# fxxJuses/MICFormer

Measured on AMD Instinct MI355X. Metric: train volumes/sec (128^3 CT+MRI pair), higher is better.
Workload: dtype bf16; 1 GPU; MicFormer base Head(embed_dim=48, depths 2-2-6-2, heads 3-6-12-24, window 2^3, 8 classes) full train step (fwd + MDiceLoss + bwd + Adam/cosine) on 128^3 CT+MR pairs, DropPath on; local_batch=2, global_batch=2, parallelism=dp1, launch=hipGraph replay (one graph)

## Files before the change

### micformer_amd/csrc/common.h

```cpp
#pragma once
#include <hip/hip_runtime.h>
#include <stdint.h>

#include "../../include/micformer_hip.h"
#include "gemm_core.h"

#define MICF_RETURN_LAUNCH()                          \
  do {                                                \
    return hipGetLastError() == hipSuccess ? MICF_OK : MICF_ELAUNCH; \
  } while (0)

namespace micf {

struct Options {
  int block_wave = 1;
  int block_recompute_h = 0;
  int block_debug = 0;
  int sample_tile = 1;
  int sample_e = -1;
  int cell_cap = -1;
  int tile_cap_hits = -1, tile_cap_cell = -1, tile_cap_voxel = -1;
};
Options& options();

struct Geo {
  int B, D, H, W;
  FastDiv fW, fH, fD;
  Geo() {}
  Geo(int B_, int D_, int H_, int W_) : B(B_), D(D_), H(H_), W(W_), fW((uint32_t)W_), fH((uint32_t)H_), fD((uint32_t)D_) {}
  __host__ __device__ int64_t tokens() const { return (int64_t)B * D * H * W; }
  __device__ __forceinline__ void decode(int t, int& b, int& d, int& h, int& w) const {
    uint32_t q, r;
    fW.divmod((uint32_t)t, q, r); w = (int)r;
    fH.divmod(q, q, r); h = (int)r;
    fD.divmod(q, q, r); d = (int)r; b = (int)q;
  }
  __device__ __forceinline__ int token(int b, int d, int h, int w) const { return ((b * D + d) * H + h) * W + w; }
};

__device__ __forceinline__ float wave_sum(float v) {
#pragma unroll
  for (int o = 32; o > 0; o >>= 1) v += __shfl_xor(v, o, 64);
  return v;
}

int colsum_atomic(const float* dy, const float* scale, int64_t rps, float* out, int64_t M, int N, hipStream_t s);

constexpr int kOffsetHidden = 16;
struct CellLists {
  int* count;
  int* ovf_count;
  int* list;
  int* ovf;
  int cap;
  float* w8;
};
struct SampleFwdSet { const float *h, *ln_g, *ln_b, *w1, *xa; float *flow, *xs; };
struct SampleBwdSet {
  const float *dxs, *h, *ln_g, *ln_b, *w1, *xa, *flow;
  float *dxa, *dh, *dln_g, *dln_b, *dw1;
  CellLists cl;
  float* partials;
};
int offset_sample_fwd_groups(const SampleFwdSet* sets, int n, int B, int D, int H, int W, int C, float eps, hipStream_t stream);
int offset_sample_bwd_groups(SampleBwdSet* sets, int n, int B, int D, int H, int W, int C, float eps, float* workspace,
                             int64_t workspace_floats, hipStream_t s, int phase = 0);
struct SampleFinishCall { const SampleBwdSet* sets; int n, B, D, H, W, C; float* workspace; int64_t workspace_floats; };
int offset_sample_finish_many(const SampleFinishCall* calls, int ncalls, hipStream_t s);

struct Conv3FwdSet { const float* x1; const float* x2; const float* w; const float* bias; float* y; float* wt; };
struct Conv3BwdSet { const float* dy; const float* w; float* wt; float* dx1; float* dx2; };
int conv3_fwd_x_groups(const Conv3FwdSet* sets, int n, int c1, int c2, int B, int D, int H, int W, int N, hipStream_t stream, int dtype,
                       int prepared, int y_zeroed);
bool conv3_fwd_x_splits(int B, int D, int H, int W, int c1, int c2);
int conv3_bwd_data_x_groups(const Conv3BwdSet* sets, int ng, int c1, int acc1, int c2, int acc2, int B, int D, int H, int W, int N,
                            hipStream_t stream, int dtype, int prepared);

int conv3_bwd_data_x(const float* dy, const float* w, float* wt, float* dx1, int c1, int acc1, float* dx2, int c2, int acc2, int B,
                     int D, int H, int W, int N, hipStream_t stream, int dtype = 0, int prepared = 0);

int64_t conv3_fwdx_workspace(int N, int c1, int c2);
int conv3_fwd_x(const float* x1, int c1, const float* x2, int c2, const float* w, const float* bias, float* y, float* wt, int B, int D,
                int H, int W, int N, hipStream_t stream, int dtype = 0, int prepared = 0);
int64_t conv3_wgradx_workspace(int B, int D, int H, int W, int N, int c1, int c2, int items = 1);
int conv3_wgradx_items(const float* const* dy, const float* const* x1, const float* const* x2, float* const* dw, float* const* dbias,
                       int n, int c1, int c2, int B, int D, int H, int W, int N, float* ws, int64_t ws_floats, hipStream_t stream,
                       int dtype);
int conv3_wgradx(const float* dy, const float* x1, int c1, const float* x2, int c2, float* dw, float* dbias, int B, int D, int H,
                 int W, int N, float* ws, int64_t ws_floats, hipStream_t stream, int dtype = 0);

}
```

### micformer_amd/csrc/conv3_wgradx.hip

```cpp
#include <cstdlib>
#include <mutex>

#include "common.h"
#include "gemm_dma.h"

namespace micf {

constexpr int wCS = 48;
constexpr int wDS = 20;
constexpr int wXS = 52;
constexpr int wPairs = 27 * (wCS / 16);
constexpr int wTPW = (wPairs + 3) / 4;
constexpr int wSlabFloats = 4 * wTPW * 256;

constexpr int kWgxItems = 12;
struct WgxArgs {
  const float* dy[kWgxItems];
  const float* x1[kWgxItems]; const float* x2[kWgxItems];
  int c1, c2;
  float* ws;
  float* bias_ws;
  int B, D, H, W, tiles_d, tiles_h, tiles_w, tiles_per_group, groups, slabs, xcd_order;
};

// ... 149 lines not shown

constexpr int wRSB = 104;
constexpr int wDYB = 40;
typedef short s16x4x __attribute__((ext_vector_type(4)));

__device__ __forceinline__ bf16x8 tr_pair(unsigned a0, unsigned a1) {
  const s16x4x lo = __builtin_amdgcn_ds_read_tr16_b64_v4i16((__attribute__((address_space(3))) s16x4x*)(uintptr_t)a0);
  const s16x4x hi = __builtin_amdgcn_ds_read_tr16_b64_v4i16((__attribute__((address_space(3))) s16x4x*)(uintptr_t)a1);
  return bf16x8{lo[0], lo[1], lo[2], lo[3], hi[0], hi[1], hi[2], hi[3]};
}

template <int TW>
__global__ void __launch_bounds__(256) conv3_wgradx_b16_kernel(WgxArgs a) {
  constexpr int TH = 64 / TW;
  constexpr int HH = TH + 2, HW = TW + 2, HALO = 3 * HH * HW;
  extern __shared__ __attribute__((aligned(16))) char smem[];
  const int tid = threadIdx.x, lane = tid & 63, wave = __builtin_amdgcn_readfirstlane(tid >> 6), li = lane & 15, lr = lane >> 4;
  int slab = blockIdx.x, group = blockIdx.y;
  const int item = blockIdx.z;
  if (a.xcd_order) {
    const int L = gridDim.x * gridDim.y;
    const int lin = slab + gridDim.x * group;
    const int logical = (lin % 8) * (L / 8) + lin / 8;
    slab = logical % gridDim.x;
    group = logical / gridDim.x;
  }
  const float* __restrict__ a_dy = a.dy[item];
  const float* __restrict__ a_x1 = a.x1[item];
  const float* __restrict__ a_x2 = a.x2[item];
  const int Cin = a.c1 + a.c2;
  const int cbase = slab * wCS;
  const int64_t DHW = (int64_t)a.D * a.H * a.W;
  const unsigned xh = (unsigned)(uintptr_t)smem, dyl = xh + HALO * wRSB;

  f32x4 acc[wTPW];
#pragma unroll
  for (int p = 0; p < wTPW; ++p) acc[p] = f32x4{0.f, 0.f, 0.f, 0.f};
  int offs[wTPW];
#pragma unroll
  for (int p = 0; p < wTPW; ++p) {
    const int pair = min(wave * wTPW + p, wPairs - 1);
    const int tap = pair / (wCS / 16), ct = pair % (wCS / 16);
    const int kd = tap / 9, kh = (tap / 3) % 3, kw = tap % 3;
    offs[p] = (((kd - 1) * HH + (kh - 1)) * HW + (kw - 1)) * wRSB + ct * 32;
  }
  unsigned abase[2][2], bbase[2][2];
#pragma unroll
  for (int ks = 0; ks < 2; ++ks)
#pragma unroll
    for (int r = 0; r < 2; ++r) {
      const int t = 8 * lr + 4 * r + (li >> 2);
      const int lh = ks * (32 / TW) + t / TW, lw = t % TW;
      abase[ks][r] = xh + (unsigned)(((1 * HH + lh + 1) * HW + lw + 1) * wRSB + 8 * (li & 3));
      bbase[ks][r] = dyl + (unsigned)((32 * ks + t) * wDYB + 8 * (li & 3));
    }
  float4 bs = make_float4(0.f, 0.f, 0.f, 0.f);

  const int ntiles = a.B * a.tiles_d * a.tiles_h * a.tiles_w;
  const int t_begin = group * a.tiles_per_group;
  const int t_end = min(ntiles, t_begin + a.tiles_per_group);
  constexpr int NQ = HALO * (wCS / 4);
  constexpr int NB = 16;
  static_assert(NQ <= 256 * NB, "one batch per tile");
  float4 v[NB], vdy;
  auto fetch = [&](int tile) {
    int q = tile;
    const int tw = q % a.tiles_w; q /= a.tiles_w;
    const int th = q % a.tiles_h; q /= a.tiles_h;
    const int d0 = q % a.tiles_d; const int b = q / a.tiles_d;
    const int h0 = th * TH, w0 = tw * TW;
#pragma unroll
    for (int u = 0; u < NB; ++u) {
      const int idx = u * 256 + tid;
      v[u] = make_float4(0.f, 0.f, 0.f, 0.f);
      if (idx < NQ) {
        const int hv = idx / (wCS / 4), g = idx % (wCS / 4);
        const int hw = hv % HW, hh = (hv / HW) % HH, hd = hv / (HW * HH);
        const int dd = d0 + hd - 1, yy = h0 + hh - 1, ww = w0 + hw - 1;
        const int c = cbase + 4 * g;
        if ((unsigned)dd < (unsigned)a.D && (unsigned)yy < (unsigned)a.H && (unsigned)ww < (unsigned)a.W && c < Cin) {
          const int64_t tok = (int64_t)b * DHW + ((int64_t)dd * a.H + yy) * a.W + ww;
          v[u] = c < a.c1 ? *reinterpret_cast<const float4*>(a_x1 + tok * a.c1 + c)
                          : *reinterpret_cast<const float4*>(a_x2 + tok * a.c2 + (c - a.c1));
        }
      }
    }
    const int tk = tid >> 2, yy = h0 + tk / TW, ww = w0 + tk % TW;
    vdy = make_float4(0.f, 0.f, 0.f, 0.f);
    if (yy < a.H && ww < a.W)
      vdy = *reinterpret_cast<const float4*>(a_dy + ((int64_t)b * DHW + ((int64_t)d0 * a.H + yy) * a.W + ww) * 16 + 4 * (tid & 3));
  };
  typedef unsigned u32x2w __attribute__((ext_vector_type(2)));
  if (t_begin < t_end) fetch(t_begin);
  for (int tile = t_begin; tile < t_end; ++tile) {
    __syncthreads();
#pragma unroll
    for (int u = 0; u < NB; ++u) {
      const int idx = u * 256 + tid;
      if (idx < NQ)
        *reinterpret_cast<u32x2w*>(smem + (idx / (wCS / 4)) * wRSB + 8 * (idx % (wCS / 4))) = u32x2w{pack_bf16(v[u].x, v[u].y), pack_bf16(v[u].z, v[u].w)};
    }
    *reinterpret_cast<u32x2w*>(smem + HALO * wRSB + (tid >> 2) * wDYB + 8 * (tid & 3)) = u32x2w{pack_bf16(vdy.x, vdy.y), pack_bf16(vdy.z, vdy.w)};
    bs.x += vdy.x; bs.y += vdy.y; bs.z += vdy.z; bs.w += vdy.w;
    __syncthreads();
    if (tile + 1 < t_end) fetch(tile + 1);
#pragma unroll
    for (int ks = 0; ks < 2; ++ks) {
      const bf16x8 bb = tr_pair(bbase[ks][0], bbase[ks][1]);
#pragma unroll
      for (int p = 0; p < wTPW; ++p) {
        const bf16x8 ba = tr_pair(abase[ks][0] + offs[p], abase[ks][1] + offs[p]);
        acc[p] = __builtin_amdgcn_mfma_f32_16x16x32_bf16(ba, bb, acc[p], 0, 0, 0);
      }
    }
  }
  float* out = a.ws + (((int64_t)item * a.slabs + slab) * a.groups + group) * wSlabFloats;
#pragma unroll
  for (int p = 0; p < wTPW; ++p)
    *reinterpret_cast<float4*>(out + ((wave * wTPW + p) * 64 + lane) * 4) = make_float4(acc[p][0], acc[p][1], acc[p][2], acc[p][3]);
  if (a.bias_ws && slab == 0) {
#pragma unroll
    for (int d = 4; d < 64; d <<= 1) {
      bs.x += __shfl_xor(bs.x, d, 64); bs.y += __shfl_xor(bs.y, d, 64); bs.z += __shfl_xor(bs.z, d, 64); bs.w += __shfl_xor(bs.w, d, 64);
    }
    __syncthreads();
    float* red = reinterpret_cast<float*>(smem);
    if (lane < 4) *reinterpret_cast<float4*>(red + (wave * 4 + lane) * 4) = bs;
    __syncthreads();
    if (tid < 16) a.bias_ws[((int64_t)item * a.groups + group) * 16 + tid] = red[tid] + red[16 + tid] + red[32 + tid] + red[48 + tid];
  }
}

struct WgxOut { float* dw[kWgxItems]; float* dbias[kWgxItems]; };
__global__ void __launch_bounds__(256) conv3_wgradx_reduce_kernel(const float* __restrict__ ws_all, const float* __restrict__ bias_all,
                                                                  WgxOut o, int Cin, int slabs, int groups) {
  __shared__ float red[256];
  const int item = blockIdx.y;
  const float* __restrict__ ws = ws_all + (int64_t)item * slabs * groups * wSlabFloats;
  const float* __restrict__ bias_ws = bias_all ? bias_all + (int64_t)item * groups * 16 : nullptr;
  float* __restrict__ dw = o.dw[item];
  float* __restrict__ dbias = o.dbias[item];
  const int el = threadIdx.x & 63, slice = threadIdx.x >> 6;
  const int64_t id = (int64_t)blockIdx.x * 64 + el;
  const int64_t per_slab = (int64_t)wPairs * 256;
  const bool main = id < per_slab * slabs;
  const bool bias = !main && bias_ws && dbias && id < per_slab * slabs + 16;
  float acc = 0.f;
  int slab = 0, e = 0;
  if (main) {
    slab = (int)(id / per_slab);
    e = (int)(id % per_slab);
    const float* p = ws + (int64_t)slab * groups * wSlabFloats + e;
    int g = slice;
    for (; g + 28 < groups; g += 32) {
      float v[8];
#pragma unroll
      for (int u = 0; u < 8; ++u) v[u] = p[(int64_t)(g + 4 * u) * wSlabFloats];
#pragma unroll
      for (int u = 0; u < 8; ++u) acc += v[u];
    }
    for (; g < groups; g += 4) acc += p[(int64_t)g * wSlabFloats];
  } else if (bias) {
    const int n = (int)(id - per_slab * slabs);
    for (int g = slice; g < groups; g += 4) acc += bias_ws[g * 16 + n];
  }
  red[threadIdx.x] = acc;
  __syncthreads();
  if (slice != 0) return;
  acc = red[el] + red[64 + el] + red[128 + el] + red[192 + el];
  if (main) {
    const int pair = e >> 8, lane = (e >> 2) & 63, v = e & 3;
    const int tap = pair / (wCS / 16), ct = pair % (wCS / 16);
    const int n = lane & 15, c = slab * wCS + ct * 16 + 4 * (lane >> 4) + v;
    if (c < Cin) dw[((int64_t)n * Cin + c) * 27 + tap] += acc;
  } else if (bias) {
    dbias[(int)(id - per_slab * slabs)] += acc;
  }
}

struct WgxPlan { int slabs, groups, tiles_per_group, tw; int64_t floats; };

static WgxPlan wgx_plan(int B, int D, int H, int W, int Cin, int items = 1) {
  WgxPlan p;
  p.tw = W >= 12 ? 16 : 8;
  const int th = 64 / p.tw;
  const int ntiles = B * D * ((H + th - 1) / th) * ((W + p.tw - 1) / p.tw);
  p.slabs = (Cin + wCS - 1) / wCS;
  constexpr int wg_target = 256;
  int groups = (wg_target + p.slabs * items - 1) / (p.slabs * items);
  if (groups < 4) groups = 4 < ntiles ? 4 : ntiles;
  if (groups > ntiles) groups = ntiles;
  p.tiles_per_group = (ntiles + groups - 1) / groups;
  p.groups = (ntiles + p.tiles_per_group - 1) / p.tiles_per_group;
  p.floats = (int64_t)p.slabs * p.groups * wSlabFloats + (int64_t)p.groups * 16;
  return p;
}

int64_t conv3_wgradx_workspace(int B, int D, int H, int W, int N, int c1, int c2, int items) {
  if (N != 16 || W < 4 || (c1 & 3) || (c2 & 3) || items < 1 || items > kWgxItems) return 0;
  return wgx_plan(B, D, H, W, c1 + c2, items).floats * items;
}

int conv3_wgradx_items(const float* const* dy, const float* const* x1, const float* const* x2, float* const* dw, float* const* dbias,
                       int n, int c1, int c2, int B, int D, int H, int W, int N, float* ws, int64_t ws_floats, hipStream_t stream,
                       int dtype) {
  const int64_t need = conv3_wgradx_workspace(B, D, H, W, N, c1, c2, n);
  if (need == 0 || !ws || ws_floats < need || !aligned16(ws)) return MICF_EUNSUPPORTED;
  const WgxPlan p = wgx_plan(B, D, H, W, c1 + c2, n);
  WgxArgs a{};
  WgxOut o{};
  bool any_bias = false;
  for (int i = 0; i < n; ++i) {
    if (!dy[i] || !x1[i] || !dw[i] || !aligned16(dy[i]) || !aligned16(x1[i]) || (x2 && x2[i] && !aligned16(x2[i]))) return MICF_EUNSUPPORTED;
    a.dy[i] = dy[i]; a.x1[i] = x1[i]; a.x2[i] = (x2 && x2[i]) ? x2[i] : x1[i];
    o.dw[i] = dw[i]; o.dbias[i] = dbias ? dbias[i] : nullptr;
    any_bias = any_bias || o.dbias[i];
  }
  a.c1 = c1; a.c2 = c2;
  a.ws = ws; a.bias_ws = any_bias ? ws + (int64_t)n * p.slabs * p.groups * wSlabFloats : nullptr;
  a.B = B; a.D = D; a.H = H; a.W = W;
  const int th = 64 / p.tw;
  a.tiles_d = D; a.tiles_h = (H + th - 1) / th; a.tiles_w = (W + p.tw - 1) / p.tw;
  a.tiles_per_group = p.tiles_per_group; a.groups = p.groups; a.slabs = p.slabs;
  a.xcd_order = ((p.slabs * p.groups) % 8 == 0) ? 1 : 0;
  static std::once_flag attr_once;
  std::call_once(attr_once, [] {
    (void)hipFuncSetAttribute(reinterpret_cast<const void*>(&conv3_wgradx_kernel<16, false>), hipFuncAttributeMaxDynamicSharedMemorySize, 80 * 1024);
    (void)hipFuncSetAttribute(reinterpret_cast<const void*>(&conv3_wgradx_kernel<8, false>), hipFuncAttributeMaxDynamicSharedMemorySize, 80 * 1024);
    (void)hipFuncSetAttribute(reinterpret_cast<const void*>(&conv3_wgradx_b16_kernel<16>), hipFuncAttributeMaxDynamicSharedMemorySize, 64 * 1024);
    (void)hipFuncSetAttribute(reinterpret_cast<const void*>(&conv3_wgradx_b16_kernel<8>), hipFuncAttributeMaxDynamicSharedMemorySize, 64 * 1024);
  });
  const dim3 grid(p.slabs, p.groups, n);
  if (p.tw == 16) {
    constexpr int HALO = 3 * (4 + 2) * (16 + 2);
    if (dtype == MICF_DTYPE_BF16) hipLaunchKernelGGL((conv3_wgradx_b16_kernel<16>), grid, dim3(256), HALO * wRSB + 64 * wDYB, stream, a);
    else hipLaunchKernelGGL((conv3_wgradx_kernel<16, false>), grid, dim3(256), sizeof(float) * (HALO * wXS + 64 * wDS), stream, a);
  } else {
    constexpr int HALO = 3 * (8 + 2) * (8 + 2);
    if (dtype == MICF_DTYPE_BF16) hipLaunchKernelGGL((conv3_wgradx_b16_kernel<8>), grid, dim3(256), HALO * wRSB + 64 * wDYB, stream, a);
    else hipLaunchKernelGGL((conv3_wgradx_kernel<8, false>), grid, dim3(256), sizeof(float) * (HALO * wXS + 64 * wDS), stream, a);
  }
  if (hipGetLastError() != hipSuccess) return MICF_ELAUNCH;
  const int64_t ne = (int64_t)wPairs * 256 * p.slabs + 16;
  hipLaunchKernelGGL(conv3_wgradx_reduce_kernel, dim3((unsigned)((ne + 63) / 64), n), dim3(256), 0, stream, ws, a.bias_ws, o,
                     c1 + c2, p.slabs, p.groups);
  return hipGetLastError() == hipSuccess ? MICF_OK : MICF_ELAUNCH;
}

int conv3_wgradx(const float* dy, const float* x1, int c1, const float* x2, int c2, float* dw, float* dbias, int B, int D, int H,
                 int W, int N, float* ws, int64_t ws_floats, hipStream_t stream, int dtype) {
  return conv3_wgradx_items(&dy, &x1, &x2, &dw, &dbias, 1, c1, c2, B, D, H, W, N, ws, ws_floats, stream, dtype);
}

}
```

### micformer_amd/csrc/linear_grouped.hip

```cpp
#include "common.h"
#include "gemm_dma.h"

namespace micf {

constexpr int kGroupMax = 32;
constexpr int kGroupChunk = 1024;

struct GItem {
  const float* a; const float* dy; const float* scale; float* out; float* dbias; float* dw;
  int M, N, K, rps;
  int tiles_i, tiles, splits, direct;
  int ldw, pad_;
  int64_t split_stride;
};
struct GArgs {
  int n;
  int end[kGroupMax];
  GItem it[kGroupMax];
};

template <bool BF16>
__global__ void __launch_bounds__(256) wgrad_grouped_kernel(const GArgs g) {
  __shared__ __attribute__((aligned(1024))) float Ps[kDmaNS * 64 * kDmaBR];
  __shared__ __attribute__((aligned(1024))) float Qs[kDmaNS * 64 * kDmaBR];
  const int total = g.end[g.n - 1];
  const int w = xcd_order(blockIdx.x, total);
  if (w >= total) return;
  int k = 0;
  while (k < g.n - 1 && w >= g.end[k]) ++k;
  const GItem& it = g.it[k];
  const int local = w - (k ? g.end[k - 1] : 0);
  const int split = local / it.tiles, t = local % it.tiles;
  const int bi = t % it.tiles_i, bj = t / it.tiles_i;
  const int i0 = bi * 64, j0 = bj * 64;
  const int tid = threadIdx.x, lane = tid & 63, wave = __builtin_amdgcn_readfirstlane(tid >> 6);
  const int li = lane & 15, lr = lane >> 4;
  const int r_begin = split * kGroupChunk;
  const int r_end = (r_begin + kGroupChunk < it.M) ? r_begin + kGroupChunk : it.M;
  const DmaOperand P{it.a, it.K, it.K}, Q{it.dy, it.N, it.N};
  const bool do_cs = (it.dbias != nullptr) && (bi == 0) && (tid < 64);

  f32x4 tot[4];
#pragma unroll
  for (int q = 0; q < 4; ++q) tot[q] = f32x4{0.f, 0.f, 0.f, 0.f};
  float ctot = 0.f;
  for (int r = r_begin; r < r_end;) {
    int seg_end = r_end;
    float s = 1.f;
    if (it.scale) {
      const int b = r / it.rps;
      s = it.scale[b];
      const int lim = (b + 1) * it.rps;
      if (lim < seg_end) seg_end = lim;
    }
    f32x4 acc[4];
#pragma unroll
    for (int q = 0; q < 4; ++q) acc[q] = f32x4{0.f, 0.f, 0.f, 0.f};
    float csum = 0.f;
    if (r != r_begin) __syncthreads();
    const int nslab = (seg_end - r) / kDmaBR;
    dma_tile_loop<true, true, kDmaNS, BF16>(P, Q, i0, j0, r, nslab, Ps, Qs, acc, do_cs, csum);
    for (int rr = r + nslab * kDmaBR; rr < seg_end; ++rr) {
      const int jq = j0 + 4 * li + wave;
      float dyv = jq < it.N ? it.dy[(int64_t)rr * it.N + jq] : 0.f;
      if constexpr (BF16) dyv = __uint_as_float(pack_bf16(dyv, 0.f) << 16);
#pragma unroll
      for (int v = 0; v < 4; ++v) {
        const int i = i0 + 16 * lr + 4 * v;
        if (i >= it.K) continue;
        float4 a4 = *reinterpret_cast<const float4*>(it.a + (int64_t)rr * it.K + i);
        if constexpr (BF16) {
          const unsigned lo = pack_bf16(a4.x, a4.y), hi = pack_bf16(a4.z, a4.w);
          a4 = make_float4(__uint_as_float(lo << 16), __uint_as_float(lo & 0xFFFF0000u), __uint_as_float(hi << 16), __uint_as_float(hi & 0xFFFF0000u));
        }
        acc[0][v] += dyv * a4.x; acc[1][v] += dyv * a4.y; acc[2][v] += dyv * a4.z; acc[3][v] += dyv * a4.w;
      }
      if (do_cs && j0 + tid < it.N) csum += it.dy[(int64_t)rr * it.N + j0 + tid];
    }
#pragma unroll
    for (int q = 0; q < 4; ++q) { tot[q][0] += s * acc[q][0]; tot[q][1] += s * acc[q][1]; tot[q][2] += s * acc[q][2]; tot[q][3] += s * acc[q][3]; }
    ctot += s * csum;
    r = seg_end;
  }
  if (do_cs && j0 + tid < it.N) atomicAdd(it.dbias + j0 + tid, ctot);
  const int j = j0 + 4 * li + wave;
  if (j >= it.N) return;
  float* base = it.direct ? it.dw : it.out + (int64_t)split * it.split_stride;
  const int ld = it.direct ? it.ldw : it.K;
#pragma unroll
  for (int v = 0; v < 4; ++v) {
    const int i = i0 + 16 * lr + 4 * v;
    if (i >= it.K) continue;
    float* p = base + (int64_t)j * ld + i;
    float4 o = make_float4(tot[0][v], tot[1][v], tot[2][v], tot[3][v]);
    if (i + 4 <= it.K) {
      if (it.direct) { const float4 old = *reinterpret_cast<const float4*>(p); o.x += old.x; o.y += old.y; o.z += old.z; o.w += old.w; }
      *reinterpret_cast<float4*>(p) = o;
    } else {
      const float e[4] = {o.x, o.y, o.z, o.w};
      for (int q = 0; q < it.K - i; ++q) p[q] = it.direct ? p[q] + e[q] : e[q];
    }
  }
}


constexpr int kB16Piece = 1024 + 64;
constexpr int kB16Stage = 4 * kB16Piece;
typedef short s16x4 __attribute__((ext_vector_type(4)));

__device__ __forceinline__ bf16x8 tr_frag(unsigned stage_piece, int li, int unit0) {
  const int r = li >> 2, u = unit0 + ((li & 3) >> 1);
  const unsigned a0 = stage_piece + (unsigned)((r * 8 + (u ^ (2 * ((r >> 1) & 1)))) * 16 + (li & 1) * 8);
  const unsigned a1 = a0 + 4 * 8 * 16;
  const s16x4 lo = __builtin_amdgcn_ds_read_tr16_b64_v4i16((__attribute__((address_space(3))) s16x4*)(uintptr_t)a0);
  const s16x4 hi = __builtin_amdgcn_ds_read_tr16_b64_v4i16((__attribute__((address_space(3))) s16x4*)(uintptr_t)a1);
  return bf16x8{lo[0], lo[1], lo[2], lo[3], hi[0], hi[1], hi[2], hi[3]};
}

__device__ __forceinline__ void dma16_b16(const uint16_t* gsrc, unsigned lds_byte) {
  dma16(reinterpret_cast<const float*>(gsrc), lds_byte);
}

__global__ void __launch_bounds__(256) wgrad_grouped_b16_kernel(const GArgs g) {
  __shared__ __attribute__((aligned(1024))) char Ps[kDmaNS * kB16Stage];
  __shared__ __attribute__((aligned(1024))) char Qs[kDmaNS * kB16Stage];
  const int total = g.end[g.n - 1];
  const int w = xcd_order(blockIdx.x, total);
  if (w >= total) return;
  int k = 0;
  while (k < g.n - 1 && w >= g.end[k]) ++k;
  const GItem& it = g.it[k];
  const int local = w - (k ? g.end[k - 1] : 0);
  const int split = local / it.tiles, t = local % it.tiles;
  const int bi = t % it.tiles_i, bj = t / it.tiles_i;
  const int i0 = bi * 64, j0 = bj * 64;
  const int tid = threadIdx.x, lane = tid & 63, wave = __builtin_amdgcn_readfirstlane(tid >> 6);
  const int li = lane & 15, lr = lane >> 4;
  const int r_begin = split * kGroupChunk;
  const int r_end = (r_begin + kGroupChunk < it.M) ? r_begin + kGroupChunk : it.M;
  const uint16_t* A = reinterpret_cast<const uint16_t*>(it.a);
  const uint16_t* DY = reinterpret_cast<const uint16_t*>(it.dy);
  const bool do_cs = (it.dbias != nullptr) && (bi == 0);

  const int srow = lane >> 3, sunit = (lane & 7) ^ (2 * ((srow >> 1) & 1));
  int xa = i0 + 8 * sunit; if (xa > it.K - 8) xa = it.K - 8;
  int xd = j0 + 8 * sunit; if (xd > it.N - 8) xd = it.N - 8;
  const unsigned pl = lds_addr(Ps) + wave * kB16Piece, ql = lds_addr(Qs) + wave * kB16Piece;
  const unsigned pf = lds_addr(Ps) + lr * kB16Piece, qf = lds_addr(Qs) + lr * kB16Piece;

  f32x4 tot[4];
#pragma unroll
  for (int q = 0; q < 4; ++q) tot[q] = f32x4{0.f, 0.f, 0.f, 0.f};
  float ctot = 0.f;
  for (int r = r_begin; r < r_end;) {
    int seg_end = r_end;
    float s = 1.f;
    if (it.scale) {
      const int b = r / it.rps;
      s = it.scale[b];
      const int lim = (b + 1) * it.rps;
      if (lim < seg_end) seg_end = lim;
    }
    f32x4 acc[4];
#pragma unroll
    for (int q = 0; q < 4; ++q) acc[q] = f32x4{0.f, 0.f, 0.f, 0.f};
    float csum = 0.f;
    if (r != r_begin) __syncthreads();
    const int nstep = (seg_end - r) / 32;
    const uint16_t* psrc = A + (int64_t)(r + 8 * wave + srow) * it.K + xa;
    const uint16_t* qsrc = DY + (int64_t)(r + 8 * wave + srow) * it.N + xd;
    const int64_t pstep = (int64_t)32 * it.K, qstep = (int64_t)32 * it.N;
#pragma unroll
    for (int st = 0; st < kDmaNS - 1; ++st) {
      if (st < nstep) {
        dma16_b16(psrc, pl + st * kB16Stage);
        dma16_b16(qsrc, ql + st * kB16Stage);
        psrc += pstep; qsrc += qstep;
      }
    }
    for (int st = 0; st < nstep; ++st) {
      wait_younger((nstep - 1 - st < kDmaNS - 2) ? nstep - 1 - st : kDmaNS - 2);
      __builtin_amdgcn_s_barrier();
      if (st + kDmaNS - 1 < nstep) {
        const int buf = (st + kDmaNS - 1) % kDmaNS;
        dma16_b16(psrc, pl + buf * kB16Stage);
        dma16_b16(qsrc, ql + buf * kB16Stage);
        psrc += pstep; qsrc += qstep;
      }
      const unsigned po = pf + (st % kDmaNS) * kB16Stage, qo = qf + (st % kDmaNS) * kB16Stage;
      const bf16x8 bb = tr_frag(qo, li, 2 * wave);
      if (do_cs) {
#pragma unroll
        for (int e = 0; e < 8; ++e) csum += __uint_as_float(((unsigned)(unsigned short)bb[e]) << 16);
      }
#pragma unroll
      for (int q = 0; q < 4; ++q) acc[q] = __builtin_amdgcn_mfma_f32_16x16x32_bf16(tr_frag(po, li, 2 * q), bb, acc[q], 0, 0, 0);
    }
#pragma unroll
    for (int q = 0; q < 4; ++q) { tot[q][0] += s * acc[q][0]; tot[q][1] += s * acc[q][1]; tot[q][2] += s * acc[q][2]; tot[q][3] += s * acc[q][3]; }
    ctot += s * csum;
    r = seg_end;
  }
  const int j = j0 + 16 * wave + li;
  if (do_cs) {
    ctot += __shfl_xor(ctot, 16, 64);
    ctot += __shfl_xor(ctot, 32, 64);
    if (lr == 0 && j < it.N) atomicAdd(it.dbias + j, ctot);
  }
  if (j >= it.N) return;
  float* base = it.direct ? it.dw : it.out + (int64_t)split * it.split_stride;
  const int ld = it.direct ? it.ldw : it.K;
#pragma unroll
  for (int q = 0; q < 4; ++q) {
    const int i = i0 + 16 * q + 4 * lr;
    if (i >= it.K) continue;
    float* p = base + (int64_t)j * ld + i;
    float4 o = make_float4(tot[q][0], tot[q][1], tot[q][2], tot[q][3]);
    if (it.direct) { const float4 old = *reinterpret_cast<const float4*>(p); o.x += old.x; o.y += old.y; o.z += old.z; o.w += old.w; }
    *reinterpret_cast<float4*>(p) = o;
  }
}

__global__ void __launch_bounds__(256) wgrad_grouped_reduce_kernel(const GArgs g) {
  const int w = blockIdx.x;
  int k = 0;
  while (k < g.n - 1 && w >= g.end[k]) ++k;
  const GItem& it = g.it[k];
  const int local = w - (k ? g.end[k - 1] : 0);
  const int64_t n4 = (int64_t)it.N * it.K / 4;
  const int64_t e = (int64_t)local * 256 + threadIdx.x;
  if (e >= n4) return;
  float* dst = it.dw + ((4 * e) / it.K) * (int64_t)it.ldw + (4 * e) % it.K;
  float4 acc = *reinterpret_cast<const float4*>(dst);
  int s = 0;
  for (; s + 4 <= it.splits; s += 4) {
    float4 v[4];
#pragma unroll
    for (int u = 0; u < 4; ++u) v[u] = *reinterpret_cast<const float4*>(it.out + (s + u) * it.split_stride + 4 * e);
#pragma unroll
    for (int u = 0; u < 4; ++u) { acc.x += v[u].x; acc.y += v[u].y; acc.z += v[u].z; acc.w += v[u].w; }
  }
  for (; s < it.splits; ++s) {
    const float4 v = *reinterpret_cast<const float4*>(it.out + s * it.split_stride + 4 * e);
    acc.x += v.x; acc.y += v.y; acc.z += v.z; acc.w += v.w;
  }
  *reinterpret_cast<float4*>(dst) = acc;
}

static bool item_ok(const micf_wgrad_item& x) {
  if (x.operand_dtype != MICF_DTYPE_F32 && x.operand_dtype != MICF_DTYPE_BF16) return false;
  if (x.operand_dtype == MICF_DTYPE_BF16) {
    if (x.M % 32 || x.N % 8 || x.K % 8 || x.N < 8 || x.K < 8) return false;
    if (x.dp_scale && x.rows_per_sample % 32) return false;
  }
  if (!x.a || !x.dy || !x.dw || x.M <= 0 || x.N < 4 || x.K < 4) return false;
  if (x.ldw != 0 && (x.ldw < x.K || x.ldw % 4)) return false;
  if (x.M >= (1LL << 30) || x.N % 4 || x.K % 4) return false;
  if ((reinterpret_cast<uintptr_t>(x.a) | reinterpret_cast<uintptr_t>(x.dy) | reinterpret_cast<uintptr_t>(x.dw)) & 15) return false;
  if (x.dp_scale && (x.rows_per_sample <= 0 || x.M % x.rows_per_sample)) return false;
  return true;
}

static int item_splits(const micf_wgrad_item& x) { return (int)((x.M + kGroupChunk - 1) / kGroupChunk); }

}

using namespace micf;

extern "C" int64_t micf_linear_bwd_weight_grouped_workspace(const micf_wgrad_item* items, int n) {
  if (!items || n <= 0) return 0;
  int64_t total = 0;
  for (int k = 0; k < n; ++k) {
    if (!item_ok(items[k])) return -1;
    const int sp = item_splits(items[k]);
    if (sp > 1) total += (int64_t)sp * items[k].N * items[k].K;
  }
  return total;
}

extern "C" int micf_linear_bwd_weight_grouped(const micf_wgrad_item* items, int n, float* workspace, int64_t workspace_floats,
                                              int dtype, micf_stream_t stream) {
  if (n < 0 || (n > 0 && !items)) return MICF_EINVAL;
  if (n == 0) return MICF_OK;
  const int64_t need = micf_linear_bwd_weight_grouped_workspace(items, n);
  if (need < 0) return MICF_EUNSUPPORTED;
  if (need > 0 && (!workspace || workspace_floats < need || (reinterpret_cast<uintptr_t>(workspace) & 15))) return MICF_EINVAL;
  hipStream_t s = (hipStream_t)stream;
  int64_t ws_off = 0;
  for (int pass = 0; pass < 2; ++pass) {
    int idx[kGroupMax], cnt = 0;
    for (int k = 0; k <= n; ++k) {
      if (k < n && (items[k].operand_dtype == MICF_DTYPE_BF16) == (pass == 1)) idx[cnt++] = k;
      if (cnt == 0 || (cnt < kGroupMax && k < n)) continue;
      GArgs g, rg;
      g.n = cnt;
      rg.n = 0;
      int blocks = 0, rblocks = 0;
      for (int q = 0; q < cnt; ++q) {
        const micf_wgrad_item& x = items[idx[q]];
        GItem& d = g.it[q];
        d.a = x.a; d.dy = x.dy; d.scale = x.dp_scale; d.dbias = x.dbias; d.dw = x.dw;
        d.M = (int)x.M; d.N = x.N; d.K = x.K; d.rps = x.dp_scale ? (int)x.rows_per_sample : (int)x.M;
        d.ldw = x.ldw > 0 ? x.ldw : x.K; d.pad_ = 0;
        d.tiles_i = ceil_div(x.K, 64);
        d.tiles = d.tiles_i * ceil_div(x.N, 64);
        d.splits = item_splits(x);
        d.direct = d.splits == 1;
        d.split_stride = (int64_t)x.N * x.K;
        d.out = d.direct ? nullptr : workspace + ws_off;
        if (!d.direct) ws_off += d.splits * d.split_stride;
        blocks += d.tiles * d.splits;
        g.end[q] = blocks;
        if (!d.direct) {
          rg.it[rg.n] = d;
          rblocks += (int)((d.split_stride / 4 + 255) / 256);
          rg.end[rg.n] = rblocks;
          ++rg.n;
        }
      }
      if (pass == 1) hipLaunchKernelGGL(wgrad_grouped_b16_kernel, dim3((blocks + 7) / 8 * 8), dim3(256), 0, s, g);
      else if (dtype == MICF_DTYPE_BF16) hipLaunchKernelGGL(wgrad_grouped_kernel<true>, dim3((blocks + 7) / 8 * 8), dim3(256), 0, s, g);
      else hipLaunchKernelGGL(wgrad_grouped_kernel<false>, dim3((blocks + 7) / 8 * 8), dim3(256), 0, s, g);
      if (hipGetLastError() != hipSuccess) return MICF_ELAUNCH;
      if (rg.n > 0) {
        hipLaunchKernelGGL(wgrad_grouped_reduce_kernel, dim3(rblocks), dim3(256), 0, s, rg);
        if (hipGetLastError() != hipSuccess) return MICF_ELAUNCH;
      }
      cnt = 0;
    }
  }
  return MICF_OK;
}
```

### micformer_amd/csrc/misc.hip

```cpp
#include <hip/hip_fp16.h>

#include "common.h"
#include <string.h>

namespace micf {

__global__ void __launch_bounds__(256) pad3d_kernel(const float* __restrict__ src, float* __restrict__ dst, int B, int D, int H,
                                                    int W, int Dp, int Hp, int Wp, int C, int64_t total) {
  for (int64_t i = (int64_t)blockIdx.x * 256 + threadIdx.x; i < total; i += (int64_t)gridDim.x * 256) {
    int64_t t = i / C; const int c = (int)(i - t * C);
    const int w = (int)(t % Wp); t /= Wp; const int h = (int)(t % Hp); t /= Hp; const int d = (int)(t % Dp); const int b = (int)(t / Dp);
    dst[i] = (d < D && h < H && w < W) ? src[((((int64_t)b * D + d) * H + h) * W + w) * C + c] : 0.f;
  }
}
__global__ void __launch_bounds__(256) crop3d_kernel(const float* __restrict__ src, float* __restrict__ dst, int B, int D, int H,
                                                     int W, int Dp, int Hp, int Wp, int C, int accumulate, int64_t total) {
  for (int64_t i = (int64_t)blockIdx.x * 256 + threadIdx.x; i < total; i += (int64_t)gridDim.x * 256) {
    int64_t t = i / C; const int c = (int)(i - t * C);
    const int w = (int)(t % W); t /= W; const int h = (int)(t % H); t /= H; const int d = (int)(t % D); const int b = (int)(t / D);
    const float v = src[((((int64_t)b * Dp + d) * Hp + h) * Wp + w) * C + c];
    dst[i] = accumulate ? dst[i] + v : v;
  }
}

__device__ __forceinline__ void ac_coord(int o, int Sin, int Sout, int& i0, int& i1, float& f) {
  const float scale = Sout > 1 ? (float)(Sin - 1) / (float)(Sout - 1) : 0.f;
  const float s = scale * (float)o;
  i0 = (int)s; if (i0 > Sin - 1) i0 = Sin - 1;
  i1 = i0 + (i0 < Sin - 1 ? 1 : 0);
  f = s - (float)i0;
}
template <bool BWD>
__global__ void __launch_bounds__(256) resize_kernel(const float* __restrict__ a, float* __restrict__ o, int B, int D, int H, int W,
                                                     int Do, int Ho, int Wo, int C, int64_t total) {
  for (int64_t i = (int64_t)blockIdx.x * 256 + threadIdx.x; i < total; i += (int64_t)gridDim.x * 256) {
    int64_t t = i / C; const int c = (int)(i - t * C);
    const int w = (int)(t % Wo); t /= Wo; const int h = (int)(t % Ho); t /= Ho; const int d = (int)(t % Do); const int b = (int)(t / Do);
    int d0, d1, h0, h1, w0, w1; float fd, fh, fw;
    ac_coord(d, D, Do, d0, d1, fd); ac_coord(h, H, Ho, h0, h1, fh); ac_coord(w, W, Wo, w0, w1, fw);
    float acc = 0.f;
    const float gv = BWD ? a[i] : 0.f;
#pragma unroll
    for (int q = 0; q < 8; ++q) {
      const int dd = (q & 4) ? d1 : d0, hh = (q & 2) ? h1 : h0, ww = (q & 1) ? w1 : w0;
      const float wt = ((q & 4) ? fd : 1.f - fd) * ((q & 2) ? fh : 1.f - fh) * ((q & 1) ? fw : 1.f - fw);
      const int64_t s = ((((int64_t)b * D + dd) * H + hh) * W + ww) * C + c;
      if (BWD) atomicAdd(o + s, wt * gv); else acc += wt * a[s];
    }
    if (!BWD) o[i] = acc;
  }
}


__global__ void __launch_bounds__(256) sw_window_kernel(const float* __restrict__ vol, float* __restrict__ win, int C, int D, int H,
                                                        int W, int rd, int rh, int rw, int z0, int y0, int x0, int64_t total) {
  for (int64_t i = (int64_t)blockIdx.x * 256 + threadIdx.x; i < total; i += (int64_t)gridDim.x * 256) {
    const int x = (int)(i % rw); int64_t r = i / rw;
    const int y = (int)(r % rh); r /= rh;
    const int z = (int)(r % rd); const int c = (int)(r / rd);
    win[i] = vol[(((int64_t)c * D + z0 + z) * H + y0 + y) * W + x0 + x];
  }
}
__global__ void __launch_bounds__(256) sw_accumulate_kernel(const float* __restrict__ pred, float* __restrict__ out,
                                                            float* __restrict__ count, int K, int D, int H, int W, int rd, int rh,
                                                            int rw, int z0, int y0, int x0, int64_t total) {
  for (int64_t i = (int64_t)blockIdx.x * 256 + threadIdx.x; i < total; i += (int64_t)gridDim.x * 256) {
    const int x = (int)(i % rw); int64_t r = i / rw;
    const int y = (int)(r % rh); r /= rh;
    const int z = (int)(r % rd); const int k = (int)(r / rd);
    const int64_t v = ((int64_t)(z0 + z) * H + y0 + y) * W + x0 + x;
    out[(int64_t)k * D * H * W + v] += pred[i];
    if (k == 0) count[v] += 1.f;
  }
}
__global__ void __launch_bounds__(256) sw_normalize_kernel(float* __restrict__ out, const float* __restrict__ count, int64_t V,
                                                           int64_t total) {
  for (int64_t i = (int64_t)blockIdx.x * 256 + threadIdx.x; i < total; i += (int64_t)gridDim.x * 256) out[i] /= count[i % V];
}

}
using namespace micf;

extern "C" int micf_abi_version(void) { return MICF_ABI_VERSION; }

micf::Options& micf::options() {
  static Options o;
  return o;
}

static int* option_slot(const char* name) {
  if (!name) return nullptr;
  Options& o = micf::options();
  const struct { const char* n; int* v; } table[] = {
      {"block_wave", &o.block_wave}, {"block_recompute_h", &o.block_recompute_h}, {"block_debug", &o.block_debug},
      {"sample_tile", &o.sample_tile}, {"sample_e", &o.sample_e}, {"cell_cap", &o.cell_cap},
      {"tile_cap_hits", &o.tile_cap_hits}, {"tile_cap_cell", &o.tile_cap_cell}, {"tile_cap_voxel", &o.tile_cap_voxel}};
  for (const auto& e : table)
    if (!strcmp(name, e.n)) return e.v;
  return nullptr;
}

extern "C" int micf_set_option(const char* name, int value) {
  int* slot = option_slot(name);
  if (!slot) return MICF_EINVAL;
  *slot = value;
  return MICF_OK;
}

extern "C" int micf_get_option(const char* name, int* value) {
  const int* slot = option_slot(name);
  if (!slot || !value) return MICF_EINVAL;
  *value = *slot;
  return MICF_OK;
}

extern "C" const char* micf_strerror(int code) {
  switch (code) {
    case MICF_OK: return "ok";
    case MICF_EINVAL: return "invalid argument (null pointer, bad size or misaligned buffer)";
    case MICF_EUNSUPPORTED: return "shape not supported by the HIP kernels";
    case MICF_ELAUNCH: return "HIP kernel launch failed";
    default: return "unknown micf error code";
  }
}

static int grid_for(int64_t total) { int64_t b = (total + 255) / 256; return (int)(b > 16384 ? 16384 : (b < 1 ? 1 : b)); }

extern "C" int micf_pad3d(const float* src, float* dst, int B, int D, int H, int W, int Dp, int Hp, int Wp, int C,
                          micf_stream_t stream) {
  if (!src || !dst || B <= 0 || D <= 0 || H <= 0 || W <= 0 || C <= 0 || Dp < D || Hp < H || Wp < W) return MICF_EINVAL;
  const int64_t total = (int64_t)B * Dp * Hp * Wp * C;
  hipLaunchKernelGGL(pad3d_kernel, dim3(grid_for(total)), dim3(256), 0, (hipStream_t)stream, src, dst, B, D, H, W, Dp, Hp, Wp, C, total);
  MICF_RETURN_LAUNCH();
}
extern "C" int micf_crop3d(const float* src, float* dst, int B, int D, int H, int W, int Dp, int Hp, int Wp, int C, int accumulate,
                           micf_stream_t stream) {
  if (!src || !dst || B <= 0 || D <= 0 || H <= 0 || W <= 0 || C <= 0 || Dp < D || Hp < H || Wp < W) return MICF_EINVAL;
  const int64_t total = (int64_t)B * D * H * W * C;
  hipLaunchKernelGGL(crop3d_kernel, dim3(grid_for(total)), dim3(256), 0, (hipStream_t)stream, src, dst, B, D, H, W, Dp, Hp, Wp, C,
                     accumulate, total);
  MICF_RETURN_LAUNCH();
}
extern "C" int micf_resize_trilinear_fwd(const float* src, float* dst, int B, int D, int H, int W, int Do, int Ho, int Wo, int C,
                                         micf_stream_t stream) {
  if (!src || !dst || B <= 0 || D <= 0 || H <= 0 || W <= 0 || Do <= 0 || Ho <= 0 || Wo <= 0 || C <= 0) return MICF_EINVAL;
  const int64_t total = (int64_t)B * Do * Ho * Wo * C;
  hipLaunchKernelGGL(resize_kernel<false>, dim3(grid_for(total)), dim3(256), 0, (hipStream_t)stream, src, dst, B, D, H, W, Do, Ho, Wo, C, total);
  MICF_RETURN_LAUNCH();
}
extern "C" int micf_resize_trilinear_bwd(const float* ddst, float* dsrc, int B, int D, int H, int W, int Do, int Ho, int Wo, int C,
                                         micf_stream_t stream) {
  if (!ddst || !dsrc || B <= 0 || D <= 0 || H <= 0 || W <= 0 || Do <= 0 || Ho <= 0 || Wo <= 0 || C <= 0) return MICF_EINVAL;
  hipStream_t s = (hipStream_t)stream;
  if (hipMemsetAsync(dsrc, 0, sizeof(float) * (size_t)B * D * H * W * C, s) != hipSuccess) return MICF_ELAUNCH;
  const int64_t total = (int64_t)B * Do * Ho * Wo * C;
  hipLaunchKernelGGL(resize_kernel<true>, dim3(grid_for(total)), dim3(256), 0, s, ddst, dsrc, B, D, H, W, Do, Ho, Wo, C, total);
  MICF_RETURN_LAUNCH();
}

extern "C" int micf_sw_window(const float* vol, float* win, int C, int D, int H, int W, int rd, int rh, int rw, int z0, int y0,
                              int x0, micf_stream_t stream) {
  if (!vol || !win || C <= 0 || rd <= 0 || rh <= 0 || rw <= 0 || z0 < 0 || y0 < 0 || x0 < 0 || z0 + rd > D || y0 + rh > H ||
      x0 + rw > W)
    return MICF_EINVAL;
  const int64_t total = (int64_t)C * rd * rh * rw;
  hipLaunchKernelGGL(sw_window_kernel, dim3(grid_for(total)), dim3(256), 0, (hipStream_t)stream, vol, win, C, D, H, W, rd, rh, rw, z0,
                     y0, x0, total);
  MICF_RETURN_LAUNCH();
}
extern "C" int micf_sw_accumulate(const float* pred, float* out, float* count, int K, int D, int H, int W, int rd, int rh, int rw,
                                  int z0, int y0, int x0, micf_stream_t stream) {
  if (!pred || !out || !count || K <= 0 || rd <= 0 || rh <= 0 || rw <= 0 || z0 < 0 || y0 < 0 || x0 < 0 || z0 + rd > D ||
      y0 + rh > H || x0 + rw > W)
    return MICF_EINVAL;
  const int64_t total = (int64_t)K * rd * rh * rw;
  hipLaunchKernelGGL(sw_accumulate_kernel, dim3(grid_for(total)), dim3(256), 0, (hipStream_t)stream, pred, out, count, K, D, H, W, rd,
                     rh, rw, z0, y0, x0, total);
  MICF_RETURN_LAUNCH();
}
extern "C" int micf_sw_normalize(float* out, const float* count, int K, int64_t V, micf_stream_t stream) {
  if (!out || !count || K <= 0 || V <= 0) return MICF_EINVAL;
  const int64_t total = (int64_t)K * V;
  hipLaunchKernelGGL(sw_normalize_kernel, dim3(grid_for(total)), dim3(256), 0, (hipStream_t)stream, out, count, V, total);
  MICF_RETURN_LAUNCH();
}

extern "C" int micf_zero(void* p, int64_t bytes, micf_stream_t stream) {
  if (!p || bytes < 0) return MICF_EINVAL;
  if (bytes == 0) return MICF_OK;
  return hipMemsetAsync(p, 0, (size_t)bytes, (hipStream_t)stream) == hipSuccess ? MICF_OK : MICF_ELAUNCH;
}

namespace micf {
__device__ __forceinline__ uint64_t mix64(uint64_t z) {
  z += 0x9E3779B97F4A7C15ull;
  z = (z ^ (z >> 30)) * 0xBF58476D1CE4E5B9ull;
  z = (z ^ (z >> 27)) * 0x94D049BB133111EBull;
  return z ^ (z >> 31);
}
__global__ void __launch_bounds__(256) drop_path_draw_kernel(uint64_t* __restrict__ rng, const float* __restrict__ keep,
                                                             float* __restrict__ out, int n, int B) {
  const uint64_t seed = rng[0], ctr = rng[1];
  for (int e = threadIdx.x; e < n * B; e += 256) {
    const float k = keep[e / B];
    const uint64_t h = mix64(mix64(seed ^ mix64(ctr)) + (uint64_t)e);
    const float u = (float)(h >> 40) * (1.0f / 16777216.0f);
    out[e] = (u < k) ? 1.0f / k : 0.0f;
  }
  __syncthreads();
  if (threadIdx.x == 0) rng[1] = ctr + 1;
}
}

extern "C" int micf_drop_path_draw(void* rng, const float* keep, float* out, int n, int B, micf_stream_t stream) {
  if (!rng || !keep || !out || n < 0 || B <= 0) return MICF_EINVAL;
  if (n == 0) return MICF_OK;
  hipLaunchKernelGGL(micf::drop_path_draw_kernel, dim3(1), dim3(256), 0, (hipStream_t)stream, static_cast<uint64_t*>(rng), keep, out, n, B);
  MICF_RETURN_LAUNCH();
}

namespace micf {
constexpr int kPrepMax = 64;
struct PrepArgs {
  int n;
  int end[kPrepMax];
  const float* src[kPrepMax]; void* dst[kPrepMax]; void* dst_t[kPrepMax];
  int rows[kPrepMax], cols[kPrepMax], bf16[kPrepMax];
};
__device__ __forceinline__ unsigned pack_bf16(float a, float b) {
  typedef __bf16 bf16x2_hw __attribute__((ext_vector_type(2)));
  typedef float f32x2_hw __attribute__((ext_vector_type(2)));
  const f32x2_hw f = {a, b};
  return __builtin_bit_cast(unsigned, __builtin_convertvector(f, bf16x2_hw));
}
__device__ __forceinline__ void prep_store4(void* base, int64_t idx, bool bf16, bool vec, int valid, float4 v) {
  if (bf16) {
    uint16_t* d = static_cast<uint16_t*>(base) + idx;
    if (vec) { *reinterpret_cast<uint2*>(d) = make_uint2(pack_bf16(v.x, v.y), pack_bf16(v.z, v.w)); return; }
    const float e[4] = {v.x, v.y, v.z, v.w};
    for (int i = 0; i < valid; ++i) d[i] = (uint16_t)(pack_bf16(e[i], 0.f) & 0xFFFFu);
  } else {
    float* d = static_cast<float*>(base) + idx;
    if (vec) { *reinterpret_cast<float4*>(d) = v; return; }
    const float e[4] = {v.x, v.y, v.z, v.w};
    for (int i = 0; i < valid; ++i) d[i] = e[i];
  }
}
__global__ void __launch_bounds__(256) weight_prep_kernel(const PrepArgs a) {
  __shared__ float t[64][65];
// ... 258 lines not shown
```

Before: 243.0 pairs/s.

## Add panel-unit bf16 wgrad kernel reusing shared operand across tiles, widen reductions

Adds an opt-in bf16 weight-gradient kernel in which each block computes a panel of up to three 64-wide output tiles. It reuses one loaded operand tile across them through a three-stage LDS pipeline, which cuts redundant global loads of the shared operand. The kernel is gated by a new 'wgrad_units' option that defaults to off. Separately, the split-K reduce and the conv3 wgrad slab reduce gain a 16-way unrolled load loop to raise memory-level parallelism when there are many splits or groups. The new kernel uses more registers and LDS per block, which may lower occupancy.

```diff
diff --git a/micformer_amd/csrc/common.h b/micformer_amd/csrc/common.h
--- a/micformer_amd/csrc/common.h
+++ b/micformer_amd/csrc/common.h
@@ -20,6 +20,7 @@
   int sample_e = -1;
   int cell_cap = -1;
   int tile_cap_hits = -1, tile_cap_cell = -1, tile_cap_voxel = -1;
+  int wgrad_units = 0;
 };
 Options& options();
 
diff --git a/micformer_amd/csrc/conv3_wgradx.hip b/micformer_amd/csrc/conv3_wgradx.hip
--- a/micformer_amd/csrc/conv3_wgradx.hip
+++ b/micformer_amd/csrc/conv3_wgradx.hip
@@ -325,6 +325,13 @@
     e = (int)(id % per_slab);
     const float* p = ws + (int64_t)slab * groups * wSlabFloats + e;
     int g = slice;
+    for (; g + 60 < groups; g += 64) {
+      float v[16];
+#pragma unroll
+      for (int u = 0; u < 16; ++u) v[u] = p[(int64_t)(g + 4 * u) * wSlabFloats];
+#pragma unroll
+      for (int u = 0; u < 16; ++u) acc += v[u];
+    }
     for (; g + 28 < groups; g += 32) {
       float v[8];
 #pragma unroll
diff --git a/micformer_amd/csrc/linear_grouped.hip b/micformer_amd/csrc/linear_grouped.hip
--- a/micformer_amd/csrc/linear_grouped.hip
+++ b/micformer_amd/csrc/linear_grouped.hip
@@ -10,7 +10,7 @@
   const float* a; const float* dy; const float* scale; float* out; float* dbias; float* dw;
   int M, N, K, rps;
   int tiles_i, tiles, splits, direct;
-  int ldw, pad_;
+  int ldw, panel;
   int64_t split_stride;
 };
 struct GArgs {
@@ -221,6 +221,159 @@
   }
 }
 
+constexpr int kUnitTiles = 3;
+constexpr int kUnitNS = 3;
+constexpr int kUnitStage = (kUnitTiles + 1) * kB16Stage;
+constexpr int kUnitMinTileBlocks = 1024;
+
+__device__ __forceinline__ void wait_unit_step(bool one_younger, int per_step) {
+  if (!one_younger) { asm volatile("s_waitcnt vmcnt(0)" ::: "memory"); return; }
+  switch (per_step) {
+    case 2: asm volatile("s_waitcnt vmcnt(2)" ::: "memory"); break;
+    case 3: asm volatile("s_waitcnt vmcnt(3)" ::: "memory"); break;
+    default: asm volatile("s_waitcnt vmcnt(4)" ::: "memory"); break;
+  }
+}
+
+__global__ void __launch_bounds__(256) __attribute__((amdgpu_waves_per_eu(3))) wgrad_units_b16_kernel(const GArgs g) {
+  __shared__ __attribute__((aligned(1024))) char Rs[kUnitNS * kUnitStage];
+  const int total = g.end[g.n - 1];
+  const int w = blockIdx.x;
+  if (w >= total) return;
+  int k = 0;
+  while (k < g.n - 1 && w >= g.end[k]) ++k;
+  const GItem& it = g.it[k];
+  const int local = w - (k ? g.end[k - 1] : 0);
+  const int split = local / it.tiles, u = local % it.tiles;
+  const bool along_k = it.panel & 1;
+  const int psz = it.panel >> 1, pa = u % it.tiles_i, ob = u / it.tiles_i;
+  const int axis_tiles = ((along_k ? it.K : it.N) + 63) / 64;
+  const int nt = psz < axis_tiles - pa * psz ? psz : axis_tiles - pa * psz;
+  const int bi0 = along_k ? pa * psz : ob, bj0 = along_k ? ob : pa * psz;
+  const int nA = along_k ? nt : 1, nD = along_k ? 1 : nt;
+  const int tid = threadIdx.x, lane = tid & 63, wave = __builtin_amdgcn_readfirstlane(tid >> 6);
+  const int li = lane & 15, lr = lane >> 4;
+  const int r_begin = split * kGroupChunk;
+  const int r_end = (r_begin + kGroupChunk < it.M) ? r_begin + kGroupChunk : it.M;
+  const uint16_t* A = reinterpret_cast<const uint16_t*>(it.a);
+  const uint16_t* DY = reinterpret_cast<const uint16_t*>(it.dy);
+  const bool do_cs = (it.dbias != nullptr) && (bi0 == 0);
+
+  const int srow = lane >> 3, sunit = (lane & 7) ^ (2 * ((srow >> 1) & 1));
+  const int xa = bi0 * 64 + 8 * sunit, xd = bj0 * 64 + 8 * sunit;
+  const unsigned wl = lds_addr(Rs) + wave * kB16Piece;
+  const unsigned fl = lds_addr(Rs) + lr * kB16Piece;
+  const unsigned dblk = nA * kB16Stage;
+
+  f32x4 tot[kUnitTiles][4];
+  float ctot[kUnitTiles];
+#pragma unroll
+  for (int p = 0; p < kUnitTiles; ++p) {
+    ctot[p] = 0.f;
+#pragma unroll
+    for (int q = 0; q < 4; ++q) tot[p][q] = f32x4{0.f, 0.f, 0.f, 0.f};
+  }
+  for (int r = r_begin; r < r_end;) {
+    int seg_end = r_end;
+    float s = 1.f;
+    if (it.scale) {
+      const int b = r / it.rps;
+      s = it.scale[b];
+      const int lim = (b + 1) * it.rps;
+      if (lim < seg_end) seg_end = lim;
+    }
+    f32x4 acc[kUnitTiles][4];
+    float csum[kUnitTiles];
+#pragma unroll
+    for (int p = 0; p < kUnitTiles; ++p) {
+      csum[p] = 0.f;
+#pragma unroll
+      for (int q = 0; q < 4; ++q) acc[p][q] = f32x4{0.f, 0.f, 0.f, 0.f};
+    }
+    if (r != r_begin) __syncthreads();
+    const int nstep = (seg_end - r) / 32;
+    const uint16_t* psrc = A + (int64_t)(r + 8 * wave + srow) * it.K + xa;
+    const uint16_t* qsrc = DY + (int64_t)(r + 8 * wave + srow) * it.N + xd;
+    const int64_t pstep = (int64_t)32 * it.K, qstep = (int64_t)32 * it.N;
+    auto issue = [&](int buf) {
+      const unsigned b = wl + buf * kUnitStage;
+#pragma unroll
+      for (int c = 0; c < kUnitTiles; ++c)
+        if (c < nA && xa + 64 * c < it.K) dma16_b16(psrc + 64 * c, b + c * kB16Stage);
+#pragma unroll
+      for (int c = 0; c < kUnitTiles; ++c)
+        if (c < nD && xd + 64 * c < it.N) dma16_b16(qsrc + 64 * c, b + dblk + c * kB16Stage);
+      psrc += pstep; qsrc += qstep;
+    };
+#pragma unroll
+    for (int st = 0; st < kUnitNS - 1; ++st)
+      if (st < nstep) issue(st);
+    for (int st = 0; st < nstep; ++st) {
+      wait_unit_step(st + 1 < nstep, nA + nD);
+      __builtin_amdgcn_s_barrier();
+      if (st + kUnitNS - 1 < nstep) issue((st + kUnitNS - 1) % kUnitNS);
+      const unsigned so = fl + (st % kUnitNS) * kUnitStage;
+      bf16x8 af[4], bb = bf16x8{0, 0, 0, 0, 0, 0, 0, 0};
+#pragma unroll
+      for (int q = 0; q < 4; ++q) af[q] = bb;
+#pragma unroll
+      for (int p = 0; p < kUnitTiles; ++p) {
+        if (p >= nt) continue;
+        const int ca = along_k ? p : 0, cb = along_k ? 0 : p;
+        const bool jv = (bj0 + cb) * 64 + 16 * wave < it.N;
+        if ((p == 0 || !along_k) && jv) {
+          bb = tr_frag(so + dblk + cb * kB16Stage, li, 2 * wave);
+          if (do_cs) {
+#pragma unroll
+            for (int e = 0; e < 8; ++e) csum[p] += __uint_as_float(((unsigned)(unsigned short)bb[e]) << 16);
+          }
+        }
+        if (p == 0 ? (jv || !along_k) : (along_k && jv)) {
+#pragma unroll
+          for (int q = 0; q < 4; ++q)
+            if ((bi0 + ca) * 64 + 16 * q < it.K) af[q] = tr_frag(so + ca * kB16Stage, li, 2 * q);
+        }
+        if (jv) {
+#pragma unroll
+          for (int q = 0; q < 4; ++q)
+            if ((bi0 + ca) * 64 + 16 * q < it.K) acc[p][q] = __builtin_amdgcn_mfma_f32_16x16x32_bf16(af[q], bb, acc[p][q], 0, 0, 0);
+        }
+      }
+    }
+#pragma unroll
+    for (int p = 0; p < kUnitTiles; ++p) {
+#pragma unroll
+      for (int q = 0; q < 4; ++q) { tot[p][q][0] += s * acc[p][q][0]; tot[p][q][1] += s * acc[p][q][1]; tot[p][q][2] += s * acc[p][q][2]; tot[p][q][3] += s * acc[p][q][3]; }
+      ctot[p] += s * csum[p];
+    }
+    r = seg_end;
+  }
+#pragma unroll
+  for (int p = 0; p < kUnitTiles; ++p) {
+    if (p >= nt) continue;
+    const int i0 = (bi0 + (along_k ? p : 0)) * 64, j0 = (bj0 + (along_k ? 0 : p)) * 64;
+    const int j = j0 + 16 * wave + li;
+    if (do_cs && (p == 0 || !along_k)) {
+      float c = ctot[p];
+      c += __shfl_xor(c, 16, 64);
+      c += __shfl_xor(c, 32, 64);
+      if (lr == 0 && j < it.N) atomicAdd(it.dbias + j, c);
+    }
+    if (j >= it.N) continue;
+    float* base = it.direct ? it.dw : it.out + (int64_t)split * it.split_stride;
+    const int ld = it.direct ? it.ldw : it.K;
+#pragma unroll
+    for (int q = 0; q < 4; ++q) {
+      const int i = i0 + 16 * q + 4 * lr;
+      if (i >= it.K) continue;
+      float* dst = base + (int64_t)j * ld + i;
+      float4 o = make_float4(tot[p][q][0], tot[p][q][1], tot[p][q][2], tot[p][q][3]);
+      if (it.direct) { const float4 old = *reinterpret_cast<const float4*>(dst); o.x += old.x; o.y += old.y; o.z += old.z; o.w += old.w; }
+      *reinterpret_cast<float4*>(dst) = o;
+    }
+  }
+}
+
 __global__ void __launch_bounds__(256) wgrad_grouped_reduce_kernel(const GArgs g) {
   const int w = blockIdx.x;
   int k = 0;
@@ -233,6 +386,13 @@
   float* dst = it.dw + ((4 * e) / it.K) * (int64_t)it.ldw + (4 * e) % it.K;
   float4 acc = *reinterpret_cast<const float4*>(dst);
   int s = 0;
+  for (; s + 16 <= it.splits; s += 16) {
+    float4 v[16];
+#pragma unroll
+    for (int u = 0; u < 16; ++u) v[u] = *reinterpret_cast<const float4*>(it.out + (s + u) * it.split_stride + 4 * e);
+#pragma unroll
+    for (int u = 0; u < 16; ++u) { acc.x += v[u].x; acc.y += v[u].y; acc.z += v[u].z; acc.w += v[u].w; }
+  }
   for (; s + 4 <= it.splits; s += 4) {
     float4 v[4];
 #pragma unroll
@@ -289,6 +449,7 @@
   int64_t ws_off = 0;
   for (int pass = 0; pass < 2; ++pass) {
     int idx[kGroupMax], cnt = 0;
+    const int unit_opt = pass == 1 ? options().wgrad_units : 0;
     for (int k = 0; k <= n; ++k) {
       if (k < n && (items[k].operand_dtype == MICF_DTYPE_BF16) == (pass == 1)) idx[cnt++] = k;
       if (cnt == 0 || (cnt < kGroupMax && k < n)) continue;
@@ -296,14 +457,25 @@
       g.n = cnt;
       rg.n = 0;
       int blocks = 0, rblocks = 0;
+      int64_t tile_blocks = 0;
+      for (int q = 0; q < cnt; ++q) tile_blocks += (int64_t)ceil_div(items[idx[q]].K, 64) * ceil_div(items[idx[q]].N, 64) * item_splits(items[idx[q]]);
+      const bool units = unit_opt == 2 || (unit_opt != 0 && tile_blocks > kUnitMinTileBlocks);
       for (int q = 0; q < cnt; ++q) {
         const micf_wgrad_item& x = items[idx[q]];
         GItem& d = g.it[q];
         d.a = x.a; d.dy = x.dy; d.scale = x.dp_scale; d.dbias = x.dbias; d.dw = x.dw;
         d.M = (int)x.M; d.N = x.N; d.K = x.K; d.rps = x.dp_scale ? (int)x.rows_per_sample : (int)x.M;
-        d.ldw = x.ldw > 0 ? x.ldw : x.K; d.pad_ = 0;
+        d.ldw = x.ldw > 0 ? x.ldw : x.K; d.panel = 0;
         d.tiles_i = ceil_div(x.K, 64);
         d.tiles = d.tiles_i * ceil_div(x.N, 64);
+        if (units) {
+          const bool along_k = x.K > x.N;
+          const int axis = along_k ? d.tiles_i : ceil_div(x.N, 64), other = along_k ? ceil_div(x.N, 64) : d.tiles_i;
+          const int npan = ceil_div(axis, kUnitTiles), psz = ceil_div(axis, npan);
+          d.panel = (along_k ? 1 : 0) | (psz << 1);
+          d.tiles_i = npan;
+          d.tiles = npan * other;
+        }
         d.splits = item_splits(x);
         d.direct = d.splits == 1;
         d.split_stride = (int64_t)x.N * x.K;
@@ -318,7 +490,8 @@
           ++rg.n;
         }
       }
-      if (pass == 1) hipLaunchKernelGGL(wgrad_grouped_b16_kernel, dim3((blocks + 7) / 8 * 8), dim3(256), 0, s, g);
+      if (units) hipLaunchKernelGGL(wgrad_units_b16_kernel, dim3((blocks + 7) / 8 * 8), dim3(256), 0, s, g);
+      else if (pass == 1) hipLaunchKernelGGL(wgrad_grouped_b16_kernel, dim3((blocks + 7) / 8 * 8), dim3(256), 0, s, g);
       else if (dtype == MICF_DTYPE_BF16) hipLaunchKernelGGL(wgrad_grouped_kernel<true>, dim3((blocks + 7) / 8 * 8), dim3(256), 0, s, g);
       else hipLaunchKernelGGL(wgrad_grouped_kernel<false>, dim3((blocks + 7) / 8 * 8), dim3(256), 0, s, g);
       if (hipGetLastError() != hipSuccess) return MICF_ELAUNCH;
diff --git a/micformer_amd/csrc/misc.hip b/micformer_amd/csrc/misc.hip
--- a/micformer_amd/csrc/misc.hip
+++ b/micformer_amd/csrc/misc.hip
@@ -94,7 +94,8 @@
   const struct { const char* n; int* v; } table[] = {
       {"block_wave", &o.block_wave}, {"block_recompute_h", &o.block_recompute_h}, {"block_debug", &o.block_debug},
       {"sample_tile", &o.sample_tile}, {"sample_e", &o.sample_e}, {"cell_cap", &o.cell_cap},
-      {"tile_cap_hits", &o.tile_cap_hits}, {"tile_cap_cell", &o.tile_cap_cell}, {"tile_cap_voxel", &o.tile_cap_voxel}};
+      {"tile_cap_hits", &o.tile_cap_hits}, {"tile_cap_cell", &o.tile_cap_cell}, {"tile_cap_voxel", &o.tile_cap_voxel},
+      {"wgrad_units", &o.wgrad_units}};
   for (const auto& e : table)
     if (!strcmp(name, e.n)) return e.v;
   return nullptr;
```

Result: no change. 243.1 pairs/s (median of 2 runs) (+0.0%).
